# FurkanOM/tf-rpn

Measured on AMD Instinct MI355X. Metric: proposal images/sec at 500x500x3 VOC batch; NMS boxes/sec, higher is better.
Workload: dtype f16x3; 1 GPU; configs[1]: 500x500x3 synthetic batch=8 per GPU, vgg16 backbone + RPN head, 9 anchors/cell, decode + NMS(300), 1xMI355X; per_gpu_batch=8, global_batch=8, img_size=500, anchors_per_image=8649, nms_topn=300, weights=random-init (seeded He-normal), parallelism=image-sharded dp1, one RCCL all-gather of proposals, nms_overlap=decode+NMS of step k on a second HIP stream, overlapping the convs of step k+1

## Files before the change

### tf_rpn_amd/csrc/conv_split_kernels.hip

```cpp
#include "split_conv.h"

namespace rpn {

template <int TH, int WN, int BBUF, int NW, bool F16, bool POOL, bool B1 = false>
__global__ void __launch_bounds__(64 * NW, NW / 2)
conv3x3_split_kernel(SplitConvArgs a, int tiles_x, int tiles_y, int n_tiles)
{
    constexpr int NT = 64 * NW;
    constexpr int WM = NW / WN;
    constexpr int MI = TH / WM;
    constexpr int NI = 2;
    constexpr int BN = WN * NI * 32;
    constexpr int HP = (TH + 2) * HW;
    constexpr int A_PIECES = HP * 4;
    constexpr int A_ROUNDS = (A_PIECES + NT - 1) / NT;
    constexpr int A_RPS = (A_ROUNDS + 2) / 3;
    constexpr int B_PIECES = 3 * BN * 4;
    constexpr int B_ROUNDS = B_PIECES / NT;
    static_assert(MI * WM == TH && B_PIECES % NT == 0, "tile shape");
    constexpr int STAGE_LD = 64 + kStagePad;
    constexpr int ABUF = HP * 4 + 4;
    constexpr int PW = TWS + 4;
    constexpr int PATCH_F = B1 ? (TH + 4) * PW * 3 : 0;
    static_assert(!B1 || (WN == 1 && POOL && BBUF == 2), "B1: the 64 -> 64 pooled instantiations only");
    constexpr int LDS_PIPE = 2 * ABUF + BBUF * B_PIECES;
    constexpr int LDS_STAGE = (NW * 32 * STAGE_LD * 4 + 15) / 16;
    constexpr int LDS_UINT4 = (LDS_PIPE > LDS_STAGE ? LDS_PIPE : LDS_STAGE) + (PATCH_F + 3) / 4;

    __shared__ uint4 lds[LDS_UINT4];
    u32x4 *As = reinterpret_cast<u32x4 *>(lds);
    u32x4 *Bs = reinterpret_cast<u32x4 *>(lds) + 2 * ABUF;

    const int tid = threadIdx.x;
    const int lane = tid & 63;
    const int wave = tid >> 6;
    const int wm = wave / WN, wn = wave % WN;
    const int lm = lane & 31, kh = lane >> 5;

    int nt, mt;
    {
        const int m_tiles = tiles_x * tiles_y * a.B;
        const int XN = n_tiles >= 8 ? 8 : (n_tiles >= 4 ? 4 : (n_tiles >= 2 ? 2 : 1)), XM = 8 / XN;
        const int NTl = (n_tiles + XN - 1) / XN;
        const int xcd = blockIdx.x & 7, slot = blockIdx.x >> 3;
        nt = (slot % NTl) * XN + (xcd % XN);
        mt = (slot / NTl) * XM + (xcd / XN);
        if (nt >= n_tiles || mt >= m_tiles) return;
    }
    const int tx = mt % tiles_x;
    mt /= tiles_x;
    const int ty = mt % tiles_y;
    const int img = mt / tiles_y;
    const int oy0 = ty * TH, ox0 = tx * TWS, n0 = nt * BN;

    const int chunks = a.Cin >> 4;
    const int steps = chunks * 3;
    const size_t in_pix_stride = (size_t)chunks * 4;
    const uint4 *__restrict__ xin = B1 ? nullptr : a.x + (size_t)img * a.H * a.W * in_pix_stride;

    constexpr int A_SLOTS = 3 * A_RPS;
    constexpr unsigned kOob = 0x80000000u;
    const __amdgpu_buffer_rsrc_t xrsrc = __builtin_amdgcn_make_buffer_rsrc(
        const_cast<uint4 *>(xin), (short)0, (int)((size_t)a.H * a.W * in_pix_stride * 16), 0x00020000);
    unsigned a_goff[A_SLOTS];
    int a_loff[A_SLOTS];
#pragma unroll
    for (int R = 0; R < (B1 ? 0 : A_SLOTS); ++R) {
        const int e = R * NT + tid;
        const int pix = e >> 2, pc = e & 3;
        const int hy = pix / HW, hx = pix - hy * HW;
        const int iy = oy0 - 1 + hy, ix = ox0 - 1 + hx;
        const bool piece = e < A_PIECES;
        const bool inimg = piece && iy >= 0 && iy < a.H && ix >= 0 && ix < a.W;
        a_loff[R] = piece ? (pix * 4 + (pc ^ ((hx >> 2) & 3))) : HP * 4;
        a_goff[R] = inimg ? (unsigned)((((size_t)iy * a.W + ix) * in_pix_stride + pc) * 16) : kOob;
    }
    u32x4 b_reg[B_ROUNDS];
    u32x4 a_reg[A_RPS];
#define RPN_LOAD_B(STEP)                                                                               \
    {                                                                                                  \
        const u32x4 *src_ = reinterpret_cast<const u32x4 *>(a.w) + ((size_t)(STEP) * 3 * a.cout_pad + n0) * 4;   \
        _Pragma("unroll") for (int i_ = 0; i_ < B_ROUNDS; ++i_) {                                      \
            const int e_ = tid + i_ * NT;                                                              \
            const int t_ = e_ / (BN * 4), rem_ = e_ - t_ * (BN * 4);                \
            b_reg[i_] = src_[(size_t)t_ * a.cout_pad * 4 + rem_];                                      \
        }                                                                                              \
    }
#define RPN_STORE_B(BUF)                                                                               \
    {                                                                                                  \
        _Pragma("unroll") for (int i_ = 0; i_ < B_ROUNDS; ++i_) {                                      \
            const int e_ = tid + i_ * NT;                                                              \
            const int t_ = e_ / (BN * 4), rem_ = e_ - t_ * (BN * 4);                                   \
            const int n_ = rem_ >> 2, pc_ = rem_ & 3;                                                  \
            Bs[(((BUF) * 3 + t_) * BN + n_) * 4 + (pc_ ^ ((n_ >> 2) & 3))] = b_reg[i_];                \
        }                                                                                              \
    }
#define RPN_LOAD_A(CHUNK, R) \
    __builtin_bit_cast(u32x4, __builtin_amdgcn_raw_buffer_load_b128(xrsrc, a_goff[R], (CHUNK) * 64, 0))

    constexpr int NBLK = (HP + 15) / 16;
    constexpr int QB = B1 ? (NBLK + NW - 1) / NW : 1;
    constexpr int QPS = (QB + 2) / 3;
    float *patchf = reinterpret_cast<float *>(lds + (LDS_PIPE > LDS_STAGE ? LDS_PIPE : LDS_STAGE));
    const int lr = lane & 15, kg = lane >> 4;
    u32x4 phi[QB], plo[QB];
    int pdst[QB];
    float b1_max = 0.0f;
    unsigned pin = 0;
    u32x4 w1hi = {0, 0, 0, 0}, w1lo = {0, 0, 0, 0};
    f32x4 b1v = {0.f, 0.f, 0.f, 0.f};
    (void)patchf; (void)lr; (void)kg; (void)pin; (void)phi; (void)plo; (void)pdst; (void)w1hi; (void)w1lo; (void)b1v;
    (void)b1_max;
#define RPN_B1_LOADW(CHUNK)                                                                            \
    {                                                                                                  \
        const u32x4 *w1_ = reinterpret_cast<const u32x4 *>(a.w1) + ((CHUNK) * 16 + lr) * 8 + kg;       \
        w1hi = w1_[0];                                                                                 \
        w1lo = w1_[4];                                                                                 \
        b1v = *reinterpret_cast<const f32x4 *>(a.b1 + (CHUNK) * 16 + 4 * kg);                          \
    }
#define RPN_B1_BLOCK(Q, BUF)                                                                           \
    {                                                                                                  \
        f32x4 c_ = {0.f, 0.f, 0.f, 0.f};                                                               \
        c_ = mfma16<F16>(w1lo, phi[Q], c_);                                                            \
        c_ = mfma16<F16>(w1hi, plo[Q], c_);                                                            \
        c_ = mfma16<F16>(w1hi, phi[Q], c_);                                                            \
        using E_ = typename Half<F16>::elem;                                                           \
        using h4_ = __attribute__((ext_vector_type(4))) E_;                                            \
        const bool in_ = (pin >> (Q)) & 1u;                                                            \
        h4_ hv_, lv_;                                                                                  \
        _Pragma("unroll") for (int r_ = 0; r_ < 4; ++r_) {                                             \
            float v_ = fmaxf(c_[r_] * a.scale1 + b1v[r_], 0.0f);                                       \
            v_ = in_ ? v_ : 0.0f;                                                                      \
            b1_max = fmaxf(b1_max, v_);                                                                \
            const E_ h_ = (E_)v_;                                                                      \
            hv_[r_] = h_;                                                                              \
            lv_[r_] = (E_)(v_ - (float)h_);                                                            \
        }                                                                                              \
        char *d_ = reinterpret_cast<char *>(As + (BUF) * ABUF);                                        \
        *reinterpret_cast<uint2 *>(d_ + pdst[Q]) = __builtin_bit_cast(uint2, hv_);                     \
        *reinterpret_cast<uint2 *>(d_ + (pdst[Q] ^ 16)) = __builtin_bit_cast(uint2, lv_);              \
    }
    if constexpr (B1) {
        const float *ximg = a.img + (size_t)img * a.H * a.W * 3;
        for (int e = tid; e < PATCH_F; e += NT) {
            const int pr = e / (PW * 3), rem = e - pr * (PW * 3);
            const int iy = oy0 - 2 + pr, ix = ox0 - 2 + rem / 3;
            patchf[e] = (iy >= 0 && iy < a.H && ix >= 0 && ix < a.W) ? ximg[((size_t)iy * a.W + ix) * 3 + rem % 3] : 0.0f;
        }
    }

    f32x16 acc[MI][NI];
#pragma unroll
    for (int i = 0; i < MI; ++i)
#pragma unroll
        for (int j = 0; j < NI; ++j)
#pragma unroll
            for (int e = 0; e < 16; ++e) acc[i][j][e] = 0.0f;

    int a_off[3];
#pragma unroll
    for (int s3 = 0; s3 < 3; ++s3) a_off[s3] = (lm + s3) * 4 + ((2 * kh) ^ (((lm + s3) >> 2) & 3));
    int b_off[NI];
#pragma unroll
    for (int j = 0; j < NI; ++j) {
        const int n = wn * (NI * 32) + j * 32 + lm;
        b_off[j] = n * 4 + ((2 * kh) ^ ((n >> 2) & 3));
    }

    if constexpr (B1) {
        RPN_LOAD_B(0);
        RPN_B1_LOADW(0);
        RPN_STORE_B(0);
        __syncthreads();
        int koff[8];
#pragma unroll
        for (int j = 0; j < 8; ++j) {
            const int k = 8 * kg + j;
            koff[j] = k < 27 ? (k / 9) * (PW * 3) + (k % 9) : -1;
        }
#pragma unroll
        for (int q = 0; q < QB; ++q) {
            const int p = (wave + NW * q) * 16 + lr;
            const bool valid = p < HP;
            const int pp = valid ? p : HP - 1;
            const int hy = pp / HW, hx = pp - hy * HW;
            const int base = (hy * PW + hx) * 3;
            float xs[8];
#pragma unroll
            for (int j = 0; j < 8; ++j) xs[j] = koff[j] >= 0 ? patchf[base + koff[j]] : 0.0f;
            phi[q] = __builtin_bit_cast(u32x4, split_piece<F16>(xs, false));
            plo[q] = __builtin_bit_cast(u32x4, split_piece<F16>(xs, true));
            const int iy = oy0 - 1 + hy, ix = ox0 - 1 + hx;
            if (iy >= 0 && iy < a.H && ix >= 0 && ix < a.W) pin |= 1u << q;
            pdst[q] = valid ? (pp * 4 + ((2 * (kg >> 1)) ^ ((hx >> 2) & 3))) * 16 + (kg & 1) * 8 : HP * 4 * 16 + (kg & 1) * 8;
        }
#pragma unroll
        for (int q = 0; q < QB; ++q) RPN_B1_BLOCK(q, 0);
    } else {
#pragma unroll
        for (int R = 0; R < A_SLOTS; ++R) As[a_loff[R]] = RPN_LOAD_A(0, R);
        RPN_LOAD_B(0);
        RPN_STORE_B(0);
    }
    __syncthreads();

    int abuf = 0, bbuf = 0;
#pragma unroll 1
    for (int chunk = 0; chunk < chunks; ++chunk) {
        const int next_chunk = chunk + 1 < chunks ? chunk + 1 : chunk;
#pragma unroll
        for (int row = 0; row < 3; ++row) {
            const int step = chunk * 3 + row;
            RPN_LOAD_B(step + 1 < steps ? step + 1 : step);
            if constexpr (B1) {
                if (row == 0) RPN_B1_LOADW(next_chunk);
            } else {
#pragma unroll
                for (int q = 0; q < A_RPS; ++q) a_reg[q] = RPN_LOAD_A(next_chunk, row * A_RPS + q);
            }
            if constexpr (NW == 4) RPN_PIN_LOADS();

            const u32x4 *arow = As + (abuf * ABUF + (wm * MI + row) * HW * 4);
#pragma unroll
            for (int s = 0; s < 3; ++s) {
                u32x4 ahi[MI], alo[MI], bhi[NI], blo[NI];
#pragma unroll
                for (int i = 0; i < MI; ++i) {
                    ahi[i] = arow[i * HW * 4 + a_off[s]];
                    alo[i] = arow[i * HW * 4 + (a_off[s] ^ 1)];
                }
#pragma unroll
                for (int j = 0; j < NI; ++j) {
                    bhi[j] = Bs[(bbuf * 3 + s) * BN * 4 + b_off[j]];
                    blo[j] = Bs[(bbuf * 3 + s) * BN * 4 + (b_off[j] ^ 1)];
                }
#pragma unroll
                for (int i = 0; i < MI; ++i)
#pragma unroll
                    for (int j = 0; j < NI; ++j) {
                        acc[i][j] = Half<F16>::mfma(alo[i], bhi[j], acc[i][j]);
                        acc[i][j] = Half<F16>::mfma(ahi[i], blo[j], acc[i][j]);
                        acc[i][j] = Half<F16>::mfma(ahi[i], bhi[j], acc[i][j]);
                    }
            }

            if (BBUF == 1) __syncthreads();
            RPN_STORE_B(BBUF == 2 ? (bbuf ^ 1) : 0);
            if constexpr (B1) {
#pragma unroll
                for (int q = row * QPS; q < (row + 1) * QPS && q < QB; ++q) RPN_B1_BLOCK(q, abuf ^ 1);
            } else {
#pragma unroll
                for (int q = 0; q < A_RPS; ++q) As[(abuf ^ 1) * ABUF + a_loff[row * A_RPS + q]] = a_reg[q];
            }
            __syncthreads();
            if (BBUF == 2) bbuf ^= 1;
        }
        abuf ^= 1;
    }

#undef RPN_LOAD_B
#undef RPN_STORE_B
#undef RPN_LOAD_A
#undef RPN_B1_LOADW
#undef RPN_B1_BLOCK
    if constexpr (B1 && F16) {
        if (a.status && !(b1_max <= 65504.0f)) atomicOr(a.status, 1u );
    }
    float *stage = reinterpret_cast<float *>(lds) + wave * (32 * STAGE_LD);
    float bias_v[NI];
#pragma unroll
    for (int j = 0; j < NI; ++j) {
        const int n = n0 + wn * (NI * 32) + j * 32 + lm;
        bias_v[j] = (a.bias && n < a.Cout) ? a.bias[n] : 0.0f;
    }
    const float act_lo = a.act == ACT_LINEAR ? -INFINITY : 0.0f;
    const float act_hi = a.act == ACT_RELU6 ? 6.0f : INFINITY;
    const int cout_chunks = a.Cout >> 4;
    const int nbase = n0 + wn * (NI * 32);
    const int pix_bytes = a.out_f32 ? a.Cout * 4 : cout_chunks * 64;
    auto store_stage = [&](int npx_log2, int oy, int oxb, int OHo, int OWo) {
        if (oy >= OHo) return;
        const long long row_off = (((long long)img * OHo + oy) * OWo + oxb) * (long long)pix_bytes;
        const __amdgpu_buffer_rsrc_t ors = __builtin_amdgcn_make_buffer_rsrc(reinterpret_cast<char *>(a.out) + row_off, (short)0,
                                                                              (OWo - oxb) * pix_bytes, 0x00020000);
        if (a.out_f32) {
            const int rounds = (16 << npx_log2) >> 6;
            const int px_l = lane >> 4, q_l = lane & 15;
            const int n = nbase + 4 * q_l;
            unsigned voff = n < a.Cout ? (unsigned)(px_l * pix_bytes + n * 4) : 0x80000000u;
#pragma unroll
            for (int rd = 0; rd < rounds; ++rd) {
                const u32x4 v = *reinterpret_cast<const u32x4 *>(&stage[(rd * 4 + px_l) * STAGE_LD + 4 * q_l]);
                __builtin_amdgcn_raw_buffer_store_b128(v, ors, voff, 0, 0);
                voff += (unsigned)(4 * pix_bytes);
            }
        } else {
            const int rounds2 = (8 << npx_log2) >> 6;
            const int px2 = lane >> 3, q2 = lane & 7;
            const int cl = q2 >> 1, hf = q2 & 1;
            const int n = nbase + cl * 16;
            unsigned voff = n < a.Cout ? (unsigned)(px2 * pix_bytes + (n >> 4) * 64 + hf * 32) : 0x80000000u;
#pragma unroll
            for (int rd = 0; rd < rounds2; ++rd) {
                float xs[8];
                const float *src = &stage[(rd * 8 + px2) * STAGE_LD + cl * 16 + hf * 8];
                const float4 v0 = *reinterpret_cast<const float4 *>(src);
                const float4 v1 = *reinterpret_cast<const float4 *>(src + 4);
                xs[0] = v0.x; xs[1] = v0.y; xs[2] = v0.z; xs[3] = v0.w;
                xs[4] = v1.x; xs[5] = v1.y; xs[6] = v1.z; xs[7] = v1.w;
                const u32x4 hi = __builtin_bit_cast(u32x4, split_piece<F16>(xs, false, a.status));
                const u32x4 lo = __builtin_bit_cast(u32x4, split_piece<F16>(xs, true, nullptr));
                __builtin_amdgcn_raw_buffer_store_b128(hi, ors, voff, 0, 0);
                __builtin_amdgcn_raw_buffer_store_b128(lo, ors, voff + 16u, 0, 0);
                voff += (unsigned)(8 * pix_bytes);
            }
        }
    };

    if constexpr (POOL) {
        static_assert(!POOL || (MI % 2 == 0), "pooling needs an even number of rows per wave");
        const int OHo = a.H >> 1, OWo = a.W >> 1;
#pragma unroll
        for (int ip = 0; ip < MI / 2; ++ip) {
#pragma unroll
            for (int j = 0; j < NI; ++j)
#pragma unroll
                for (int e2 = 0; e2 < 8; ++e2) {
                    const float v0 = fmaxf(acc[2 * ip][j][2 * e2], acc[2 * ip][j][2 * e2 + 1]);
                    const float v1 = fmaxf(acc[2 * ip + 1][j][2 * e2], acc[2 * ip + 1][j][2 * e2 + 1]);
                    const int m2 = (e2 & 1) + 4 * (e2 >> 1) + 2 * kh;
                    stage[m2 * STAGE_LD + j * 32 + lm] = fminf(fmaxf(fmaxf(v0, v1) * a.out_scale + bias_v[j], act_lo), act_hi);
                }
            wave_sync();
            store_stage(4, (oy0 + wm * MI + 2 * ip) >> 1, ox0 >> 1, OHo, OWo);
            wave_sync();
        }
    } else {
#pragma unroll
        for (int i = 0; i < MI; ++i) {
#pragma unroll
            for (int j = 0; j < NI; ++j)
#pragma unroll
                for (int e = 0; e < 16; ++e) {
                    const int m = (e & 3) + 8 * (e >> 2) + 4 * kh;
                    stage[m * STAGE_LD + j * 32 + lm] = fminf(fmaxf(acc[i][j][e] * a.out_scale + bias_v[j], act_lo), act_hi);
                }
            wave_sync();
            store_stage(5, oy0 + wm * MI + i, ox0, a.H, a.W);
            wave_sync();
        }
    }
}

template <int TH, int WN, int BBUF, bool F16, bool POOL, int NW = 4>
static hipError_t launch_split_variant(const SplitConvArgs &a, hipStream_t s)
{
    const SplitGrid g = split_grid(a.B, a.H, a.W, a.Cout, TH, WN * 64);
    const long long nblocks = 8 * g.slots;
    if (!g.valid || nblocks > 0x7fffffffll) return hipErrorInvalidValue;
    hipLaunchKernelGGL((conv3x3_split_kernel<TH, WN, BBUF, NW, F16, POOL>), dim3((unsigned)nblocks), dim3(64 * NW), 0,
                       s, a, g.tiles_x, g.tiles_y, g.n_tiles);
    return hipGetLastError();
}


int conv3x3_split_tile(int B, int H, int W, int Cout, bool pool)
{
    static const int force_tile = RPN_LAB_KNOB("RPN_SPLIT_TILE", 0);
    const long long mt8 = (long long)((W + 31) / 32) * ((H + 7) / 8) * B;
    const long long mt4 = (long long)((W + 31) / 32) * ((H + 3) / 4) * B;
    const int nt128 = (Cout + 127) / 128;
    int tile;
    if (Cout <= 64) tile = 81;
    else if (mt8 * nt128 >= 512) tile = 82;
    else if (mt4 * nt128 >= 512 || pool) tile = 42;
    else tile = 41;
    if (force_tile && Cout > 64 && !(pool && force_tile == 41)) tile = force_tile;
    return tile;
}

template <bool F16, bool POOL>
static hipError_t launch_split_tiles(const SplitConvArgs &a, hipStream_t s)
{
    const int tile = conv3x3_split_tile(a.B, a.H, a.W, a.Cout, POOL);
    int bbuf = (tile == 82) ? 1 : 2;
#ifdef RPN_LAB
    static const int force_bbuf = RPN_LAB_KNOB("RPN_SPLIT_BBUF", 0);
    if (force_bbuf) bbuf = force_bbuf;
    if (tile == 82 && bbuf == 2) bbuf = 1;
    static const int force_waves = RPN_LAB_KNOB("RPN_SPLIT_WAVES", 0);
    if (tile == 82 && force_waves == 8) return launch_split_variant<8, 2, 1, F16, POOL, 8>(a, s);
    static const int small_mode = RPN_LAB_KNOB("RPN_SPLIT_SMALL", 0);
    if constexpr (!POOL) {
        const long long mt4 = (long long)((a.W + 31) / 32) * ((a.H + 3) / 4) * a.B;
        const int nt128 = (a.Cout + 127) / 128;
        if (tile == 41 && small_mode == 2 && mt4 * nt128 >= 256) return launch_split_variant<4, 2, 2, F16, false, 8>(a, s);
    }
#endif
    switch (tile * 10 + bbuf) {
        case 821: return launch_split_variant<8, 2, 1, F16, POOL>(a, s);
        case 812: return launch_split_variant<8, 1, 2, F16, POOL>(a, s);
        case 422: return launch_split_variant<4, 2, 2, F16, POOL>(a, s);
        case 412: if constexpr (!POOL) return launch_split_variant<4, 1, 2, F16, false>(a, s); else break;
#ifdef RPN_LAB
        case 811: return launch_split_variant<8, 1, 1, F16, POOL>(a, s);
        case 421: return launch_split_variant<4, 2, 1, F16, POOL>(a, s);
        case 411: if constexpr (!POOL) return launch_split_variant<4, 1, 1, F16, false>(a, s); else break;
#endif
        default: break;
    }
    return hipErrorInvalidValue;
}

hipError_t launch_conv3x3_split(const void *x, const void *w, const float *bias, void *out, int B, int H, int W,
                                int Cin, int Cout, int cout_pad, float out_scale, int act, bool out_f32, bool f16,
                                bool pool, hipStream_t s, bool ktree)
{
    if (ktree) return hipErrorInvalidValue;
    if (Cin % 16 != 0 || Cout % 16 != 0 || cout_pad % 64 != 0 || act == ACT_SIGMOID) return hipErrorInvalidValue;
    SplitConvArgs a{};
    a.status = range_status();
    a.x = (const uint4 *)x; a.w = (const uint4 *)w; a.bias = bias; a.out = out;
    a.B = B; a.H = H; a.W = W; a.Cin = Cin; a.Cout = Cout; a.cout_pad = cout_pad;
    a.out_scale = out_scale; a.act = act; a.out_f32 = out_f32 ? 1 : 0;
    return with_bool(f16, [&](auto F16) {
        return with_bool(pool, [&](auto POOL) { return launch_split_tiles<F16(), POOL()>(a, s); });
    });
}

hipError_t launch_vgg_block1(const float *img, const void *w1, const float *b1, float scale1, const void *w2,
                             const float *b2, float scale2, void *out, int B, int H, int W, bool f16, hipStream_t s)
{
    if (B < 1 || H < 2 || W < 2) return hipErrorInvalidValue;
    SplitConvArgs a{};
    a.status = range_status();
    a.x = nullptr; a.w = (const uint4 *)w2; a.bias = b2; a.out = out;
    a.B = B; a.H = H; a.W = W; a.Cin = 64; a.Cout = 64; a.cout_pad = 64;
    a.out_scale = scale2; a.act = ACT_RELU; a.out_f32 = 0;
    a.img = img; a.w1 = (const uint4 *)w1; a.b1 = b1; a.scale1 = scale1;
    const SplitGrid g = split_grid(B, H, W, 64, 8, 64);
    const long long nblocks = 8 * g.slots;
    if (nblocks > 0x7fffffffll) return hipErrorInvalidValue;
    with_bool(f16, [&](auto F16) {
        hipLaunchKernelGGL((conv3x3_split_kernel<8, 1, 2, 4, F16(), true, true>), dim3((unsigned)nblocks), dim3(256), 0, s, a,
                           g.tiles_x, g.tiles_y, g.n_tiles);
    });
    return hipGetLastError();
}

}
```

Measured before the change: 3103 images/s.

## Interleave fused first-layer MFMA blocks into the B1 conv main loop schedule

```diff
diff --git a/tf_rpn_amd/csrc/conv_split_kernels.hip b/tf_rpn_amd/csrc/conv_split_kernels.hip
--- a/tf_rpn_amd/csrc/conv_split_kernels.hip
+++ b/tf_rpn_amd/csrc/conv_split_kernels.hip
@@ -101,14 +101,20 @@
     constexpr int NBLK = (HP + 15) / 16;
     constexpr int QB = B1 ? (NBLK + NW - 1) / NW : 1;
     constexpr int QPS = (QB + 2) / 3;
+    static_assert(!B1 || QPS <= 2, "B1: at most one first-layer block under each of taps 1 and 2");
     float *patchf = reinterpret_cast<float *>(lds + (LDS_PIPE > LDS_STAGE ? LDS_PIPE : LDS_STAGE));
     const int lr = lane & 15, kg = lane >> 4;
     u32x4 phi[QB], plo[QB];
     int pdst[QB];
+    using bh = typename Half<F16>::elem;
+    using bh4 = __attribute__((ext_vector_type(4))) bh;
     float b1_max = 0.0f;
     unsigned pin = 0;
     u32x4 w1hi = {0, 0, 0, 0}, w1lo = {0, 0, 0, 0};
     f32x4 b1v = {0.f, 0.f, 0.f, 0.f};
+    constexpr int PATCH_R = B1 ? (PATCH_F + NT - 1) / NT : 1;
+    float patch_v[PATCH_R];
+    (void)patch_v;
     (void)patchf; (void)lr; (void)kg; (void)pin; (void)phi; (void)plo; (void)pdst; (void)w1hi; (void)w1lo; (void)b1v;
     (void)b1_max;
 #define RPN_B1_LOADW(CHUNK)                                                                            \
@@ -118,18 +124,14 @@
         w1lo = w1_[4];                                                                                 \
         b1v = *reinterpret_cast<const f32x4 *>(a.b1 + (CHUNK) * 16 + 4 * kg);                          \
     }
-#define RPN_B1_BLOCK(Q, BUF)                                                                           \
-    {                                                                                                  \
-        f32x4 c_ = {0.f, 0.f, 0.f, 0.f};                                                               \
-        c_ = mfma16<F16>(w1lo, phi[Q], c_);                                                            \
-        c_ = mfma16<F16>(w1hi, plo[Q], c_);                                                            \
-        c_ = mfma16<F16>(w1hi, phi[Q], c_);                                                            \
+#define RPN_B1_FINISH(Q, BUF, C)                                                                       \
+    {                                                                                                  \
         using E_ = typename Half<F16>::elem;                                                           \
         using h4_ = __attribute__((ext_vector_type(4))) E_;                                            \
         const bool in_ = (pin >> (Q)) & 1u;                                                            \
         h4_ hv_, lv_;                                                                                  \
         _Pragma("unroll") for (int r_ = 0; r_ < 4; ++r_) {                                             \
-            float v_ = fmaxf(c_[r_] * a.scale1 + b1v[r_], 0.0f);                                       \
+            float v_ = fmaxf((C)[r_] * a.scale1 + b1v[r_], 0.0f);                                      \
             v_ = in_ ? v_ : 0.0f;                                                                      \
             b1_max = fmaxf(b1_max, v_);                                                                \
             const E_ h_ = (E_)v_;                                                                      \
@@ -140,12 +142,40 @@
         *reinterpret_cast<uint2 *>(d_ + pdst[Q]) = __builtin_bit_cast(uint2, hv_);                     \
         *reinterpret_cast<uint2 *>(d_ + (pdst[Q] ^ 16)) = __builtin_bit_cast(uint2, lv_);              \
     }
+#define RPN_B1_CUT() __builtin_amdgcn_sched_barrier(0)
+#define RPN_B1_ELEM(R, Q, C, HV, LV)         \
+    {                                                                                                  \
+        float v_ = fmaxf((C)[R] * a.scale1 + b1v[R], 0.0f);                                            \
+        v_ = ((pin >> (Q)) & 1u) ? v_ : 0.0f;                                                          \
+        b1_max = fmaxf(b1_max, v_);                                                                    \
+        const bh h_ = (bh)v_;                                                                          \
+        (HV)[R] = h_;                                                                                  \
+        (LV)[R] = (bh)(v_ - (float)h_);                                                                \
+    }
+#define RPN_B1_STORE(Q, BUF, HV, LV)                                                                   \
+    {                                                                                                  \
+        char *d_ = reinterpret_cast<char *>(As + (BUF) * ABUF);                                        \
+        *reinterpret_cast<uint2 *>(d_ + pdst[Q]) = __builtin_bit_cast(uint2, HV);                      \
+        *reinterpret_cast<uint2 *>(d_ + (pdst[Q] ^ 16)) = __builtin_bit_cast(uint2, LV);               \
+    }
+#define RPN_B1_BLOCK(Q, BUF)                                                                           \
+    {                                                                                                  \
+        f32x4 c_ = {0.f, 0.f, 0.f, 0.f};                                                               \
+        c_ = mfma16<F16>(w1lo, phi[Q], c_);                                                            \
+        c_ = mfma16<F16>(w1hi, plo[Q], c_);                                                            \
+        c_ = mfma16<F16>(w1hi, phi[Q], c_);                                                            \
+        RPN_B1_FINISH(Q, BUF, c_);                                                                     \
+    }
     if constexpr (B1) {
         const float *ximg = a.img + (size_t)img * a.H * a.W * 3;
-        for (int e = tid; e < PATCH_F; e += NT) {
+#pragma unroll
+        for (int r = 0; r < PATCH_R; ++r) {
+            const int e = tid + r * NT;
             const int pr = e / (PW * 3), rem = e - pr * (PW * 3);
             const int iy = oy0 - 2 + pr, ix = ox0 - 2 + rem / 3;
-            patchf[e] = (iy >= 0 && iy < a.H && ix >= 0 && ix < a.W) ? ximg[((size_t)iy * a.W + ix) * 3 + rem % 3] : 0.0f;
+            const bool in = e < PATCH_F && iy >= 0 && iy < a.H && ix >= 0 && ix < a.W;
+            const float v = ximg[in ? ((size_t)iy * a.W + ix) * 3 + rem % 3 : 0];
+            patch_v[r] = in ? v : 0.0f;
         }
     }
 
@@ -170,6 +200,9 @@
     if constexpr (B1) {
         RPN_LOAD_B(0);
         RPN_B1_LOADW(0);
+#pragma unroll
+        for (int r = 0; r < PATCH_R; ++r)
+            if (tid + r * NT < PATCH_F) patchf[tid + r * NT] = patch_v[r];
         RPN_STORE_B(0);
         __syncthreads();
         int koff[8];
@@ -196,6 +229,7 @@
         }
 #pragma unroll
         for (int q = 0; q < QB; ++q) RPN_B1_BLOCK(q, 0);
+        RPN_B1_LOADW(chunks > 1 ? 1 : 0);
     } else {
 #pragma unroll
         for (int R = 0; R < A_SLOTS; ++R) As[a_loff[R]] = RPN_LOAD_A(0, R);
@@ -205,6 +239,8 @@
     __syncthreads();
 
     int abuf = 0, bbuf = 0;
+    u32x4 alo_c[MI], bhi_c[NI], blo_c[NI];
+    (void)alo_c; (void)bhi_c; (void)blo_c;
 #pragma unroll 1
     for (int chunk = 0; chunk < chunks; ++chunk) {
         const int next_chunk = chunk + 1 < chunks ? chunk + 1 : chunk;
@@ -212,15 +248,86 @@
         for (int row = 0; row < 3; ++row) {
             const int step = chunk * 3 + row;
             RPN_LOAD_B(step + 1 < steps ? step + 1 : step);
-            if constexpr (B1) {
-                if (row == 0) RPN_B1_LOADW(next_chunk);
-            } else {
+            if constexpr (!B1) {
 #pragma unroll
                 for (int q = 0; q < A_RPS; ++q) a_reg[q] = RPN_LOAD_A(next_chunk, row * A_RPS + q);
             }
             if constexpr (NW == 4) RPN_PIN_LOADS();
 
             const u32x4 *arow = As + (abuf * ABUF + (wm * MI + row) * HW * 4);
+            if constexpr (B1) {
+                const u32x4 *brow = Bs + bbuf * 3 * BN * 4;
+                u32x4 ahi[MI], bhi_n[NI];
+                if (row == 0) {
+#pragma unroll
+                    for (int i = 0; i < MI; ++i) alo_c[i] = arow[i * HW * 4 + (a_off[0] ^ 1)];
+                }
+#pragma unroll
+                for (int j = 0; j < NI; ++j) bhi_c[j] = brow[b_off[j]];
+#pragma unroll
+                for (int s = 0; s < 3; ++s) {
+                    const int q1 = row * QPS + s - 1;
+                    const bool blk = s >= 1 && s - 1 < QPS && q1 < QB;
+                    const int qq = blk ? q1 : 0;
+                    f32x4 c1 = {0.f, 0.f, 0.f, 0.f};
+                    bh4 hv1, lv1;
+                    ahi[0] = arow[a_off[s]];
+                    if (s == 0) blo_c[0] = brow[b_off[0] ^ 1];
+                    if (blk) c1 = mfma16<F16>(w1lo, phi[qq], c1);
+                    acc[0][0] = Half<F16>::mfma(alo_c[0], bhi_c[0], acc[0][0]);
+                    RPN_B1_CUT();
+                    if (s == 0) blo_c[1] = brow[b_off[1] ^ 1];
+                    ahi[1] = arow[HW * 4 + a_off[s]];
+                    if (blk) c1 = mfma16<F16>(w1hi, plo[qq], c1);
+                    acc[0][1] = Half<F16>::mfma(alo_c[0], bhi_c[1], acc[0][1]);
+                    RPN_B1_CUT();
+                    if (blk) c1 = mfma16<F16>(w1hi, phi[qq], c1);
+                    acc[1][0] = Half<F16>::mfma(alo_c[1], bhi_c[0], acc[1][0]);
+                    RPN_B1_CUT();
+                    acc[1][1] = Half<F16>::mfma(alo_c[1], bhi_c[1], acc[1][1]);
+                    RPN_B1_CUT();
+                    const bool a_next = s < 2 || row < 2;
+                    const u32x4 *arow_n = s < 2 ? arow : arow + HW * 4;
+                    const int a_off_n = a_off[s < 2 ? s + 1 : 0] ^ 1;
+                    if (a_next) alo_c[0] = arow_n[a_off_n];
+                    acc[0][0] = Half<F16>::mfma(ahi[0], blo_c[0], acc[0][0]);
+                    if (blk) RPN_B1_ELEM(0, qq, c1, hv1, lv1);
+                    RPN_B1_CUT();
+                    acc[0][1] = Half<F16>::mfma(ahi[0], blo_c[1], acc[0][1]);
+                    RPN_B1_CUT();
+                    if (a_next) alo_c[1] = arow_n[HW * 4 + a_off_n];
+                    acc[1][0] = Half<F16>::mfma(ahi[1], blo_c[0], acc[1][0]);
+                    if (blk) RPN_B1_ELEM(1, qq, c1, hv1, lv1);
+                    RPN_B1_CUT();
+                    acc[1][1] = Half<F16>::mfma(ahi[1], blo_c[1], acc[1][1]);
+                    RPN_B1_CUT();
+                    if (s == 2) {
+                        RPN_STORE_B(bbuf ^ 1);
+                        RPN_B1_CUT();
+                    }
+                    if (s < 2) {
+                        bhi_n[0] = brow[(s + 1) * BN * 4 + b_off[0]];
+                        blo_c[0] = brow[(s + 1) * BN * 4 + (b_off[0] ^ 1)];
+                    }
+                    acc[0][0] = Half<F16>::mfma(ahi[0], bhi_c[0], acc[0][0]);
+                    if (blk) RPN_B1_ELEM(2, qq, c1, hv1, lv1);
+                    RPN_B1_CUT();
+                    if (s < 2) bhi_n[1] = brow[(s + 1) * BN * 4 + b_off[1]];
+                    acc[0][1] = Half<F16>::mfma(ahi[0], bhi_c[1], acc[0][1]);
+                    RPN_B1_CUT();
+                    if (s < 2) blo_c[1] = brow[(s + 1) * BN * 4 + (b_off[1] ^ 1)];
+                    acc[1][0] = Half<F16>::mfma(ahi[1], bhi_c[0], acc[1][0]);
+                    if (blk) RPN_B1_ELEM(3, qq, c1, hv1, lv1);
+                    RPN_B1_CUT();
+                    acc[1][1] = Half<F16>::mfma(ahi[1], bhi_c[1], acc[1][1]);
+                    if (blk) RPN_B1_STORE(qq, abuf ^ 1, hv1, lv1);
+                    RPN_B1_CUT();
+                    if (s < 2) {
+                        bhi_c[0] = bhi_n[0];
+                        bhi_c[1] = bhi_n[1];
+                    }
+                }
+            } else {
 #pragma unroll
             for (int s = 0; s < 3; ++s) {
                 u32x4 ahi[MI], alo[MI], bhi[NI], blo[NI];
@@ -243,12 +350,12 @@
                         acc[i][j] = Half<F16>::mfma(ahi[i], bhi[j], acc[i][j]);
                     }
             }
+            }
 
             if (BBUF == 1) __syncthreads();
-            RPN_STORE_B(BBUF == 2 ? (bbuf ^ 1) : 0);
+            if constexpr (!B1) RPN_STORE_B(BBUF == 2 ? (bbuf ^ 1) : 0);
             if constexpr (B1) {
-#pragma unroll
-                for (int q = row * QPS; q < (row + 1) * QPS && q < QB; ++q) RPN_B1_BLOCK(q, abuf ^ 1);
+                if (row == 2) RPN_B1_LOADW(chunk + 2 < chunks ? chunk + 2 : chunks - 1);
             } else {
 #pragma unroll
                 for (int q = 0; q < A_RPS; ++q) As[(abuf ^ 1) * ABUF + a_loff[row * A_RPS + q]] = a_reg[q];
@@ -264,6 +371,10 @@
 #undef RPN_LOAD_A
 #undef RPN_B1_LOADW
 #undef RPN_B1_BLOCK
+#undef RPN_B1_FINISH
+#undef RPN_B1_ELEM
+#undef RPN_B1_STORE
+#undef RPN_B1_CUT
     if constexpr (B1 && F16) {
         if (a.status && !(b1_max <= 65504.0f)) atomicOr(a.status, 1u );
     }
```

Result: no change. 3116 images/s, median of 6 (+0.4%).
